# chenhuims/DistributedDeepLearningSpark

Measured on AMD Instinct MI355X. Metric: images/sec (whole node) ResNet-50 ImageNet-shape at 1/2/4/8 MI355X, higher is better.
Workload: dtype bf16; 1 GPU; model=resnet50, global_batch=256, image=224, per_gpu_batch=256, parallelism=dp1, optimizer=sgd-momentum, buckets=4

## Files before the change

distributeddeeplearningspark_amd/csrc/kernels/gemm_stream.hip:

```cpp
#include "ddl_gemm_kernel.h"

namespace ddl {
namespace gst {

constexpr int THREADS = 256;
constexpr int BM = 64;
constexpr int LDS_BUDGET = 80 * 1024;
typedef __attribute__((address_space(3))) void lds_t;

template <int WN, int K>
struct Cfg {
  static constexpr int NB = 4 * WN;
  static constexpr int RN = WN / 16;
  static constexpr int KS = K / 32;
  static constexpr int CPR = K / 8;
  static constexpr int TILE = BM * K * 2;
  static constexpr int D = TILE / 1024 / 4;
  static constexpr int OCPR = NB / 8;
  static constexpr int STAGE = BM * NB * 2;
  static constexpr int RPP = THREADS / OCPR;
  static constexpr int S = BM / RPP;
  static constexpr int NBUF_FIT = (LDS_BUDGET - STAGE) / TILE;
  static constexpr int NBUF = NBUF_FIT > 4 ? 4 : NBUF_FIT;
  static constexpr int LDS = NBUF * TILE + STAGE;
  static_assert(NBUF >= 2, "A ring needs two buffers");
  static_assert(D >= 1 && OCPR >= 8 && RPP >= 1 && BM % RPP == 0, "shape");
  static_assert((NBUF - 1) * (D + S) <= 63, "vmcnt range");
  static_assert(4 * 2 * OCPR * 8 * 4 <= STAGE, "stats reduction fits in the staging buffer");
};

template <int CPR>
__device__ __forceinline__ int sw(int r) {
  if constexpr (CPR == 8) return (r >> 1) & 7;
  else return r & 15;
}

template <int N>
__device__ __forceinline__ void wait_vm() {
  __builtin_amdgcn_s_waitcnt((N & 15) | ((N >> 4) << 14) | 0x0F70);
}

template <class CF>
__device__ __forceinline__ void wait_tile(int younger_store_tiles) {
  constexpr int base = (CF::NBUF - 1) * CF::D;
  switch (younger_store_tiles) {
    case 0: wait_vm<base>(); break;
    case 1: wait_vm<base + CF::S>(); break;
    case 2: wait_vm<base + 2 * CF::S>(); break;
    default: wait_vm<base + 3 * CF::S>(); break;
  }
}

template <class CF>
__device__ __forceinline__ void stage_a(const bf16_t* __restrict__ A, long lda, int M, int m0, char* slot, int w,
                                        int lane) {
#pragma unroll
  for (int i = 0; i < CF::D; ++i) {
    const int blk = i * 4 + w;
    const int u = blk * 64 + lane;
    const int r = u / CF::CPR, cp = u % CF::CPR;
    const int c = cp ^ sw<CF::CPR>(r);
    const int gr = min(m0 + r, M - 1);
    const bf16_t* src = A + (long)gr * lda + c * 8;
    const uint32_t dst = __builtin_amdgcn_readfirstlane((uint32_t) reinterpret_cast<uintptr_t>((lds_t*)(slot + blk * 1024)));
    asm volatile("s_mov_b32 m0, %1\n\tglobal_load_lds_dwordx4 %0, off" ::"v"(src), "s"(dst) : "memory", "m0");
  }
}

}

typedef __attribute__((ext_vector_type(2))) unsigned u32x2_t;
typedef __attribute__((ext_vector_type(4))) unsigned u32x4_t;
__device__ __forceinline__ u32x4_t ald128(const void* p) {
  u32x4_t v;
  asm volatile("global_load_dwordx4 %0, %1, off" : "=v"(v) : "v"(p) : "memory");
  return v;
}
__device__ __forceinline__ u32x2_t ald64(const void* p) {
  u32x2_t v;
  asm volatile("global_load_dwordx2 %0, %1, off" : "=v"(v) : "v"(p) : "memory");
  return v;
}
__device__ __forceinline__ unsigned ald32(const void* p) {
  unsigned v;
  asm volatile("global_load_dword %0, %1, off" : "=v"(v) : "v"(p) : "memory");
  return v;
}
__device__ __forceinline__ unsigned ald16(const void* p) {
  unsigned v;
  asm volatile("global_load_ushort %0, %1, off" : "=v"(v) : "v"(p) : "memory");
  return v;
}
__device__ __forceinline__ unsigned ald8(const void* p) {
  unsigned v;
  asm volatile("global_load_ubyte %0, %1, off" : "=v"(v) : "v"(p) : "memory");
  return v;
}
template <bool ASM> __device__ __forceinline__ u32x4_t sld128(const void* p) {
  if constexpr (ASM) return ald128(p);
  return *reinterpret_cast<const u32x4_t*>(p);
}
template <bool ASM> __device__ __forceinline__ u32x2_t sld64(const void* p) {
  if constexpr (ASM) return ald64(p);
  return *reinterpret_cast<const u32x2_t*>(p);
}
template <bool ASM> __device__ __forceinline__ unsigned sld32(const void* p) {
  if constexpr (ASM) return ald32(p);
  return *reinterpret_cast<const uint32_t*>(p);
}
template <bool ASM> __device__ __forceinline__ unsigned sld16(const void* p) {
  if constexpr (ASM) return ald16(p);
  return *reinterpret_cast<const uint16_t*>(p);
}
template <bool ASM> __device__ __forceinline__ unsigned sld8(const void* p) {
  if constexpr (ASM) return ald8(p);
  return *reinterpret_cast<const uint8_t*>(p);
}


template <int WN, int K, int BMODE, bool RES, int BNR = 0>
__global__ __launch_bounds__(gst::THREADS, 2) void gemm_stream_kernel(const GemmParams p) {
  using namespace gst;
  using CF = Cfg<WN, K>;
  constexpr bool kAsmSide = true;
  __shared__ __attribute__((aligned(16))) char smem[CF::LDS];
  char* const stg = smem + CF::NBUF * CF::TILE;
  const int lane = threadIdx.x & 63, w = threadIdx.x >> 6;
  const int n0 = blockIdx.y * CF::NB;
  const int mt = (p.M + BM - 1) / BM;
  const int nloc = ((int)blockIdx.x < mt) ? (mt - 1 - (int)blockIdx.x) / (int)gridDim.x + 1 : 0;
  const bf16_t* __restrict__ A = reinterpret_cast<const bf16_t*>(p.a);

  bf16x8 bfr[CF::RN][CF::KS];
  {
    const bf16_t* __restrict__ B = reinterpret_cast<const bf16_t*>(p.b);
#pragma unroll
    for (int rn = 0; rn < CF::RN; ++rn)
#pragma unroll
      for (int ks = 0; ks < CF::KS; ++ks) {
        const int n = n0 + WN * w + 16 * rn + (lane & 15);
        const int k = 32 * ks + 8 * (lane >> 4);
        if constexpr (BMODE == OP_KC) {
          bfr[rn][ks] = *reinterpret_cast<const bf16x8*>(B + (long)n * p.ldb + k);
        } else {
          s16x8 v;
#pragma unroll
          for (int j = 0; j < 8; ++j) v[j] = (short)B[(long)(k + j) * p.ldb + n];
          bfr[rn][ks] = __builtin_bit_cast(bf16x8, v);
        }
      }
  }
  float bias_r[CF::RN][4];
#pragma unroll
  for (int rn = 0; rn < CF::RN; ++rn) {
    const float4 bv = p.bias ? *reinterpret_cast<const float4*>(p.bias + n0 + WN * w + 16 * rn + 4 * (lane >> 4))
                             : make_float4(0.f, 0.f, 0.f, 0.f);
    bias_r[rn][0] = bv.x;
    bias_r[rn][1] = bv.y;
    bias_r[rn][2] = bv.z;
    bias_r[rn][3] = bv.w;
  }
  wait_vm<0>();
  auto tile_m0 = [&](int i) { return min((int)blockIdx.x + i * (int)gridDim.x, mt - 1) * BM; };

#pragma unroll
  for (int s = 0; s < CF::NBUF - 1; ++s) stage_a<CF>(A, p.lda, p.M, tile_m0(s), smem + s * CF::TILE, w, lane);

  float s1[8], s2[8];
#pragma unroll
  for (int e = 0; e < 8; ++e) s1[e] = s2[e] = 0.f;
  const int oc = threadIdx.x % CF::OCPR, orow = threadIdx.x / CF::OCPR;
  float bmu[8];
  float bsc[BNR == 2 ? 8 : 1], bsh[BNR == 2 ? 8 : 1];
  if constexpr (BNR != 0) {
    const float4 a = *reinterpret_cast<const float4*>(p.bnr_mean + n0 + oc * 8);
    const float4 b = *reinterpret_cast<const float4*>(p.bnr_mean + n0 + oc * 8 + 4);
    bmu[0] = a.x; bmu[1] = a.y; bmu[2] = a.z; bmu[3] = a.w;
    bmu[4] = b.x; bmu[5] = b.y; bmu[6] = b.z; bmu[7] = b.w;
  }
  if constexpr (BNR == 2) {
    const float4 a0 = *reinterpret_cast<const float4*>(p.bnr_scale + n0 + oc * 8);
    const float4 a1 = *reinterpret_cast<const float4*>(p.bnr_scale + n0 + oc * 8 + 4);
    const float4 b0 = *reinterpret_cast<const float4*>(p.bnr_shift + n0 + oc * 8);
    const float4 b1 = *reinterpret_cast<const float4*>(p.bnr_shift + n0 + oc * 8 + 4);
    bsc[0] = a0.x; bsc[1] = a0.y; bsc[2] = a0.z; bsc[3] = a0.w; bsc[4] = a1.x; bsc[5] = a1.y; bsc[6] = a1.z; bsc[7] = a1.w;
    bsh[0] = b0.x; bsh[1] = b0.y; bsh[2] = b0.z; bsh[3] = b0.w; bsh[4] = b1.x; bsh[5] = b1.y; bsh[6] = b1.z; bsh[7] = b1.w;
  }
  bf16_t* __restrict__ Cout = reinterpret_cast<bf16_t*>(p.c);

  for (int i = 0; i < nloc; ++i) {
    const int m0 = tile_m0(i);
    u32x2_t rres[BM / 16][CF::RN];
    unsigned rmk32[BM / 16];
    u32x2_t rmk64[CF::RN == 4 ? BM / 16 : 1];
    unsigned rodd_bits = 0u;
    const bool has_mask = p.resid_mask != nullptr;
    if constexpr (RES) {
#pragma unroll
      for (int mb = 0; mb < BM / 16; ++mb) {
        const int m = min(m0 + 16 * mb + (lane & 15), p.M - 1);
        long rrow = m;
        if (p.rsub_h) {
          int rn_, ri_, rj_;
          pix_decompose((uint32_t)m, p.rsub_h, p.rsub_w, rn_, ri_, rj_);
          const bool rodd = (ri_ | rj_) & 1;
          rodd_bits |= (rodd ? 1u : 0u) << mb;
// ... 77 lines not shown
          v[3] += (mk & 8u) ? __uint_as_float(rv.y & 0xffff0000u) : 0.f;
        }
        if (p.relu == ACT_RELU) {
#pragma unroll
          for (int e = 0; e < 4; ++e) v[e] = fmaxf(v[e], 0.f);
        }
        *reinterpret_cast<uint2*>(stg + r * (CF::NB * 2) + (((nl >> 3) ^ sw<CF::OCPR>(r)) << 4) + (nl & 7) * 2) =
            make_uint2(pack_bf16x2(v[0], v[1]), pack_bf16x2(v[2], v[3]));
      }
    }
    __builtin_amdgcn_s_waitcnt(0xC07F);
    __builtin_amdgcn_s_barrier();

    if constexpr (kAsmSide && BNR) {
      wait_vm<CF::D>();
      __builtin_amdgcn_sched_barrier(0);
#pragma unroll
      for (int ps = 0; ps < CF::S; ++ps) {
        asm volatile("" : "+v"(bx[ps]));
        if constexpr (BNR == 1) asm volatile("" : "+v"(bm8[ps]));
      }
    }
#pragma unroll
    for (int ps = 0; ps < CF::S; ++ps) {
      const int r = orow + ps * CF::RPP;
      const int m = m0 + r;
      const uint4 v = *reinterpret_cast<const uint4*>(stg + r * (CF::NB * 2) + ((oc ^ sw<CF::OCPR>(r)) << 4));
      if (m < p.M) {
        *reinterpret_cast<uint4*>(Cout + (long)m * p.ldc + n0 + oc * 8) = v;
        if constexpr (BNR) {
          const uint32_t wv[4] = {v.x, v.y, v.z, v.w};
          const uint32_t xv[4] = {bx[ps].x, bx[ps].y, bx[ps].z, bx[ps].w};
          uint32_t bmk = 0xffu;
          if constexpr (BNR == 1) bmk = p.bnr_mask ? bm8[ps] : 0xffu;
#pragma unroll
          for (int q = 0; q < 4; ++q) {
#pragma unroll
            for (int h = 0; h < 2; ++h) {
              const int e = 2 * q + h;
              const float xe = __uint_as_float(h ? (xv[q] & 0xffff0000u) : (xv[q] << 16));
              bool keep;
              if constexpr (BNR == 2) keep = xe * bsc[e] + bsh[e] > 0.f;
              else keep = (bmk >> e) & 1u;
              const float d = keep ? __uint_as_float(h ? (wv[q] & 0xffff0000u) : (wv[q] << 16)) : 0.f;
              s1[e] += d;
              s2[e] += d * (xe - bmu[e]);
            }
          }
        } else if (p.stats) {
          const uint32_t wv[4] = {v.x, v.y, v.z, v.w};
#pragma unroll
          for (int q = 0; q < 4; ++q) {
            const float lo = __uint_as_float(wv[q] << 16), hi = __uint_as_float(wv[q] & 0xffff0000u);
            s1[2 * q] += lo;
            s2[2 * q] += lo * lo;
            s1[2 * q + 1] += hi;
            s2[2 * q + 1] += hi * hi;
          }
        }
      }
    }
  }
  wait_vm<0>();

  if (p.stats) {
#pragma unroll
    for (int o = CF::OCPR; o < 64; o <<= 1)
#pragma unroll
      for (int e = 0; e < 8; ++e) {
        s1[e] += __shfl_xor(s1[e], o, 64);
        s2[e] += __shfl_xor(s2[e], o, 64);
      }
    __syncthreads();
    float* red = reinterpret_cast<float*>(stg);
    if (lane < CF::OCPR) {
#pragma unroll
      for (int e = 0; e < 8; ++e) {
        red[(w * CF::OCPR + lane) * 16 + e] = s1[e];
        red[(w * CF::OCPR + lane) * 16 + 8 + e] = s2[e];
      }
    }
    __syncthreads();
    float* st = p.stats + (long)(blockIdx.x % kStatShards) * 2 * p.N;
    for (int t = threadIdx.x; t < CF::NB; t += THREADS) {
      const int ch = t >> 3, e = t & 7;
      float a = 0.f, b = 0.f;
#pragma unroll
      for (int ww = 0; ww < 4; ++ww) {
        a += red[(ww * CF::OCPR + ch) * 16 + e];
        b += red[(ww * CF::OCPR + ch) * 16 + 8 + e];
      }
      atomicAdd(st + n0 + t, a);
      atomicAdd(st + p.N + n0 + t, b);
    }
  }
}

namespace {

int num_cus() {
  static int cus = 0;
  if (!cus) {
    int dev = 0;
    (void)hipGetDevice(&dev);
    if (hipDeviceGetAttribute(&cus, hipDeviceAttributeMultiprocessorCount, dev) != hipSuccess || cus <= 0) cus = 256;
  }
  return cus;
}

template <int WN, int K, int BMODE>
int launch_ws(const GemmParams& p, hipStream_t s) {
  using CF = gst::Cfg<WN, K>;
  constexpr bool kRes = !(WN == 64 && K == 128);
  constexpr bool kBnr = CF::NB <= (K >= 256 ? 64 : 128);
  const int panels = p.N / CF::NB;
  const int mt = (p.M + gst::BM - 1) / gst::BM;
  const int gx = std::max(1, std::min(mt, 2 * num_cus() / std::max(1, panels)));
  if (p.bnr_x && p.bnr_scale) {
    if constexpr (kBnr) {
      if (p.resid) return (int)hipErrorInvalidValue;
      hipLaunchKernelGGL((gemm_stream_kernel<WN, K, BMODE, false, 2>), dim3(gx, panels), dim3(gst::THREADS), 0, s, p);
    } else {
      return (int)hipErrorInvalidValue;
    }
  } else if (p.bnr_x) {
    if constexpr (kBnr && kRes) {
      if (p.resid)
        hipLaunchKernelGGL((gemm_stream_kernel<WN, K, BMODE, true, 1>), dim3(gx, panels), dim3(gst::THREADS), 0, s, p);
      else
        hipLaunchKernelGGL((gemm_stream_kernel<WN, K, BMODE, false, 1>), dim3(gx, panels), dim3(gst::THREADS), 0, s, p);
    } else if constexpr (kBnr) {
      if (p.resid) return (int)hipErrorInvalidValue;
      hipLaunchKernelGGL((gemm_stream_kernel<WN, K, BMODE, false, 1>), dim3(gx, panels), dim3(gst::THREADS), 0, s, p);
    } else {
      return (int)hipErrorInvalidValue;
    }
  } else if (p.resid) {
    if constexpr (kRes)
      hipLaunchKernelGGL((gemm_stream_kernel<WN, K, BMODE, true>), dim3(gx, panels), dim3(gst::THREADS), 0, s, p);
    else
      return (int)hipErrorInvalidValue;
  } else {
    hipLaunchKernelGGL((gemm_stream_kernel<WN, K, BMODE, false>), dim3(gx, panels), dim3(gst::THREADS), 0, s, p);
  }
  return (int)hipGetLastError();
}

template <int WN, int BMODE>
int launch_k(const GemmParams& p, hipStream_t s) {
  switch (p.K) {
    case 64: return launch_ws<WN, 64, BMODE>(p, s);
    case 128: return launch_ws<WN, 128, BMODE>(p, s);
    default:
      if constexpr (WN <= 32) return launch_ws<WN, 256, BMODE>(p, s);
      return (int)hipErrorInvalidValue;
  }
}

template <int BMODE>
int launch_panel(const GemmParams& p, int nb, hipStream_t s) {
  switch (nb) {
    case 64: return launch_k<16, BMODE>(p, s);
    case 128: return launch_k<32, BMODE>(p, s);
    default: return launch_k<64, BMODE>(p, s);
  }
}

}

int gemm_stream_panel(int N, int K) {
  if (K != 64 && K != 128 && K != 256) return 0;
  const int max_nb = K == 256 ? 128 : 256;
  for (int nb = max_nb; nb >= 64; nb >>= 1)
    if (N % nb == 0 && (N == nb || nb == max_nb)) return nb;
  return 0;
}

int launch_gemm_stream(const GemmParams& p, int epi, hipStream_t s) {
  int nb = gemm_stream_panel(p.N, p.K);
  if (p.resid && p.K == 128 && nb == 256) nb = 128;
  if (p.bnr_x && nb > (p.K >= 256 ? 64 : 128)) nb = p.K >= 256 ? 64 : 128;
  const bool ok = nb && epi == EPI_BF16 && p.a_mode == OP_KC && (p.b_mode == OP_KC || p.b_mode == OP_RC) &&
                  !p.om.enabled && !p.aux && !p.drop_thresh && (p.relu == ACT_NONE || p.relu == ACT_RELU) &&
                  p.beta == 0.f && p.k_split >= p.K && p.lda % 8 == 0 && p.ldc % 8 == 0 &&
                  (p.b_mode == OP_RC || p.ldb % 8 == 0) && (!p.resid || p.ldr % 4 == 0) &&
                  ((uintptr_t)p.a % 16 == 0) && ((uintptr_t)p.c % 16 == 0) &&
                  (p.b_mode == OP_RC || (uintptr_t)p.b % 16 == 0) && (!p.resid || (uintptr_t)p.resid % 8 == 0) &&
                  (!p.bnr_x || (p.stats && (uintptr_t)p.bnr_x % 16 == 0 && (uintptr_t)p.bnr_mean % 16 == 0)) &&
                  (!p.bnr_scale || (p.bnr_shift && !p.resid && (uintptr_t)p.bnr_scale % 16 == 0 &&
                                    (uintptr_t)p.bnr_shift % 16 == 0));
  if (!ok) return (int)hipErrorInvalidValue;
  return p.b_mode == OP_KC ? launch_panel<OP_KC>(p, nb, s) : launch_panel<OP_RC>(p, nb, s);
}

}
```

distributeddeeplearningspark_amd/ops/gemm.py:

```python
from __future__ import annotations

import math

import torch

from . import determinism as _det
from ._native import C

KC, RC, KC_GATHER, RC_GATHER, RC_TAPS, KC_GATHER8, RC_GATHER8 = 0, 1, 2, 3, 4, 5, 6
EPI_BF16, EPI_F32, EPI_F32_ATOMIC = 0, 1, 2
TILE256 = 4
TILE_STREAM = 5
TILE_CONV3 = 6
_TILES = {0: (128, 128), 1: (128, 64), 2: (64, 128), 3: (64, 64), TILE256: (256, 256), TILE_STREAM: (64, 256),
          TILE_CONV3: (224, 128)}
_ONE_PER_CU = (TILE256,)
_CU = 256
import os as _os

_USE256 = "auto"


_USE_STREAM = "1"
_TILE_FILL = 2.0
_WT_MIN_M = 4096
_LINEAR_WGRAD_ROUNDS = 1.0
_SPLIT_ROUNDS = 2.0


def stream_panel(N: int, K: int) -> int:
    if K not in (64, 128, 256):
        return 0
    max_nb = 128 if K == 256 else 256
    nb = max_nb
    while nb >= 64:
        if N % nb == 0 and (N == nb or nb == max_nb):
            return nb
        nb //= 2
    return 0


def use_stream(M, N, K, a_mode, b_mode, epi, lda, ldc, *, outmap=None, aux=None, drop_p=0.0, relu=0, beta=0.0,
               resid=None, ldr=0) -> bool:
    if _USE_STREAM == "0" or a_mode != KC or b_mode not in (KC, RC) or epi != EPI_BF16:
        return False
    if outmap is not None or aux is not None or drop_p or int(relu) > ACT_RELU or beta:
        return False
    if M < 16384 or not stream_panel(N, K) or lda % 8 or ldc % 8 or (resid is not None and ldr % 4):
        return False
    return True


def use_tile256(M: int, N: int, K: int, a_mode: int, b_mode: int, epi: int) -> bool:
    if _USE256 == "0" or a_mode > RC or b_mode > RC or K % 64 or M < 128 or N < 128:
        return False
    tiles = math.ceil(M / 256) * math.ceil(N / 256)
    if _USE256 == "1":
        return tiles >= _CU // 2
    return epi == EPI_BF16 and tiles >= 4 * _CU and K >= 4096


def choose_tile(M: int, N: int, bn_cap: int = 128) -> int:
    bn = 128 if (N > 64 and bn_cap >= 128) else 64
    bm = 128 if M > 64 else 64
    if bm == 128 and bn == 128 and math.ceil(M / 128) * math.ceil(N / 128) < _TILE_FILL * _CU:
        bm = 64 if M <= N else 128
        bn = 64 if M > N else 128
    for tid, (tm, tn) in _TILES.items():
        if (tm, tn) == (bm, bn):
            return tid
    return 3


def choose_split(M: int, N: int, K: int, tile: int, allow: bool, rounds: float | None = None) -> int:
    kfull = max(64, math.ceil(K / 64) * 64)
    if not allow:
        return kfull
    bm, bn = _TILES[tile]
    tiles = math.ceil(M / bm) * math.ceil(N / bn)
    per_cu = 1 if tile in _ONE_PER_CU else 2
    if tiles >= per_cu * _CU or K < 1024:
        return kfull
    splits = min(math.ceil((rounds or _SPLIT_ROUNDS) * per_cu * _CU / tiles), max(1, K // 512))
    ks = math.ceil(K / splits / 64) * 64
    return max(64, ks)


def gemm(a, b, c, M, N, K, a_mode, b_mode, lda, ldb, ldc, epi, *, alpha=1.0, beta=0.0, bias=None, resid=None,
         ldr=0, relu=False, geom=None, outmap=None, b_kdiv=0, b_tap_stride=0, stats=None, tile=None, k_split=None,
         bn_cap=128, aux=None, drop_p=0.0, drop_seed=0, split_rounds=None, resid_mask=None, bnr=None, rsub=None,
         slabs=None, defer_slabs=False):
    if tile is None:
        if use_stream(M, N, K, a_mode, b_mode, epi, lda, ldc, outmap=outmap, aux=aux, drop_p=drop_p, relu=relu,
                      beta=beta, resid=resid, ldr=ldr):
            tile = TILE_STREAM
        elif outmap is None and bnr is None and use_tile256(M, N, K, a_mode, b_mode, epi):
            tile = TILE256
        elif epi == EPI_F32 and a_mode <= RC and b_mode <= RC and big_wgrad(M, N, K) and _SPLITK_SLABS_MODE != "0":
            tile = 0
        else:
            tile = choose_tile(M, N, bn_cap)
    if (k_split is None and tile == 0 and epi == EPI_F32 and a_mode == RC and b_mode == RC and big_wgrad(M, N, K)
            and _SPLITK_SLABS_MODE == "auto" and slabs is not False):
        k_split = slab_split(M, N, K)
    if k_split is None:
        k_split = choose_split(M, N, K, tile, allow=(epi != EPI_BF16), rounds=split_rounds)
    split_stride = 0
    if k_split < K and epi != EPI_F32 and _det.enabled():
        k_split = max(64, math.ceil(K / 64) * 64)
    out, slab_beta = c, None
    if epi == EPI_F32 and k_split < K:
        if beta not in (0.0, 1.0):
            raise ValueError("split-K fp32 gemm supports beta in {0,1} (beta=0 needs a zeroed C)")
        auto = _SPLITK_SLABS_MODE == "auto" and tile == 0 and big_wgrad(M, N, K) and math.ceil(K / k_split) <= 32
        use_slabs = (_det.enabled() or _SPLITK_SLABS or auto) if slabs is None else (slabs or _det.enabled())
        if tile in (0, 1, 2, 3) + _ONE_PER_CU and use_slabs:
            splits = math.ceil(K / k_split)
            out, split_stride, slab_beta, ldc_c = _slab_workspace(splits * M * N, c.device), M * N, beta, ldc
            ldc, beta = N, 0.0
# ... 173 lines not shown
```

distributeddeeplearningspark_amd/csrc/kernels/conv3x3.hip:

```cpp
#include "ddl_gemm_kernel.h"
#include "ddl_ops.h"

namespace ddl {
namespace {

constexpr int C3_MAX_HALO_ROWS = 384;

struct Conv3Tiling {
  int img, rows, w;
  int P;
  int hh, ww;
  int hr, hr_pad;
  int tiles_img, tiles_row;
};

template <int BN, int EPI, int NB, int FR = 8>
__global__ __launch_bounds__(NTHREADS, 2) void conv3x3_halo_kernel(const GemmParams p, const Conv3Tiling t) {
  constexpr int RN = BN / 32;
  constexpr int B_BYTES = BN * BK * 2;
  extern __shared__ __attribute__((aligned(16))) char smem[];
  char* halo = smem;
  char* bring = smem + t.hr_pad * 128;

  const ConvGeom& g = p.g;
  const int H = g.hi, W = g.wi, C = g.c, N = g.n;
  const int tiles_n = (p.N + BN - 1) / BN;
  int bid, split;
  grid_tile(bid, split);
  const int tp = bid / tiles_n, tn = bid - tp * tiles_n;
  const int n0 = tn * BN;
  const int timg = tp / t.tiles_row, trow = tp - timg * t.tiles_row;
  const int img0 = timg * t.img, oy0 = trow * t.rows;
  const long m0 = ((long)img0 * H + oy0) * W;
  const int mend = (int)min((long)p.M, m0 + t.P);

  const int lane = threadIdx.x & 63, wid = threadIdx.x >> 6;
  const int wm = wid >> 1, wn = wid & 1;
  const int wn0 = wn * (BN / 2);

  int abase[FR];
#pragma unroll
  for (int i = 0; i < FR; ++i) {
    const int px = wm * (16 * FR) + 16 * i + (lane & 15);
    if (px < t.P) {
      const int im = px / (t.rows * t.w);
      const int rem = px - im * t.rows * t.w;
      const int oy = rem / t.w, ox = rem - oy * t.w;
      abase[i] = im * t.hh * t.ww + oy * t.ww + ox;
    } else {
      abase[i] = 0;
    }
  }

  Operand<BN, OP_KC> B;
  B.init(p.b, p.ldb, p.N, n0, p.K, g);

  const bf16_t* x = reinterpret_cast<const bf16_t*>(p.a);
  const int halo_instr = t.hr_pad / 32;
  constexpr int kMaxHaloInstr = C3_MAX_HALO_ROWS / 32;
  int hofs[kMaxHaloInstr];
#pragma unroll
  for (int j = 0; j < kMaxHaloInstr; ++j) {
    hofs[j] = -1;
    const int piece = wid + 4 * j;
    const int h = piece * 8 + (lane >> 3);
    if (j < halo_instr && h < t.hr) {
      const int chunk = (lane & 7) ^ (h & 6);
      const int im = h / (t.hh * t.ww);
      const int rem = h - im * t.hh * t.ww;
      const int hy = rem / t.ww, hx = rem - hy * t.ww;
      const int n = img0 + im, iy = oy0 + hy - 1, ix = hx - 1;
      if (n < N && (unsigned)iy < (unsigned)H && (unsigned)ix < (unsigned)W)
        hofs[j] = ((n * H + iy) * W + ix) * C + chunk * 8;
    }
  }
  const uint32_t halo_lds = lds_addr(halo) + (uint32_t)__builtin_amdgcn_readfirstlane(wid) * 1024u;
  auto stage_halo = [&](int kc) {
#pragma unroll
    for (int j = 0; j < kMaxHaloInstr; ++j) {
      if (j < halo_instr) {
        const void* src = hofs[j] >= 0 ? (const void*)(x + hofs[j] + kc * 64) : (const void*)ddl_zero_page;
        dma16(src, halo_lds + (uint32_t)(j * 4096));
      }
    }
  };
  auto stage_b = [&](int s, char* buf) {
    const int kc = s / 9, tap = s - kc * 9;
    B.dma(buf, tap * C + kc * 64, g, 0, 0, wid);
  };

  f32x4 acc[FR][RN];
#pragma unroll
  for (int i = 0; i < FR; ++i)
#pragma unroll
    for (int j = 0; j < RN; ++j) acc[i][j] = f32x4{0.f, 0.f, 0.f, 0.f};

  const int steps = (C / 64) * 9;
  stage_halo(0);
  stage_b(0, bring);
  for (int s = 0; s < steps; ++s) {
    const int kc = s / 9, tap = s - kc * 9;
    wait_vmcnt<0>();
    __builtin_amdgcn_s_barrier();
    if (s + 1 < steps) stage_b(s + 1, bring + ((s + 1) % NB) * B_BYTES);
    const char* lb = bring + (s % NB) * B_BYTES;
    const int r = tap / 3, c3 = tap - r * 3;
    const int toff = r * t.ww + c3;
#pragma unroll
    for (int kk = 0; kk < BK / 32; ++kk) {
      bf16x8 af[FR], bfr[RN];
#pragma unroll
      for (int j = 0; j < RN; ++j) bfr[j] = B.frag(lb, kk, j, wn0, lane);
#pragma unroll
      for (int i = 0; i < FR; ++i) {
        const int row = abase[i] + toff;
        const int ch = kk * 4 + (lane >> 4);
        af[i] = *reinterpret_cast<const bf16x8*>(halo + row * 128 + ((ch ^ (row & 6)) << 4));
      }
#pragma unroll
      for (int i = 0; i < FR; ++i)
#pragma unroll
        for (int j = 0; j < RN; ++j) acc[i][j] = mfma16x16x32(bfr[j], af[i], acc[i][j]);
    }
    if (NB == 2 || tap == 8) {
      asm volatile("s_waitcnt lgkmcnt(0)" ::: "memory");
      __builtin_amdgcn_s_barrier();
    }
    if (tap == 8 && s + 1 < steps) stage_halo(kc + 1);
  }

  gemm_epilogue<FR, RN, EPI>(p, acc, m0 + wm * (16 * FR), n0 + wn0, lane, bid, mend);
}

Conv3Tiling plan(const GemmParams& p, int max_px = 256) {
  const ConvGeom& g = p.g;
  Conv3Tiling t{};
  const int H = g.hi, W = g.wi;
  t.w = W;
  if (H * W <= max_px) {
    t.rows = H;
    t.img = std::max(1, std::min(max_px / (H * W), C3_MAX_HALO_ROWS / ((H + 2) * (W + 2))));
  } else {
    t.img = 1;
    t.rows = 0;
    for (int r = std::min(H, max_px / std::max(W, 1)); r >= 1; --r)
      if (H % r == 0 && (r + 2) * (W + 2) <= C3_MAX_HALO_ROWS) { t.rows = r; break; }
  }
  t.P = t.img * t.rows * t.w;
  t.hh = t.rows + 2;
  t.ww = W + 2;
  t.hr = t.img * t.hh * t.ww;
  t.hr_pad = (t.hr + 31) / 32 * 32;
  t.tiles_row = t.rows > 0 ? H / t.rows : 0;
  t.tiles_img = (g.n + t.img - 1) / t.img;
  return t;
}

template <int BN, int EPI, int NB, int FR>
int launch_fr(const GemmParams& p, const Conv3Tiling& t, hipStream_t s) {
  const int blocks = t.tiles_img * t.tiles_row * ((p.N + BN - 1) / BN);
  const size_t lds = (size_t)t.hr_pad * 128 + NB * BN * BK * 2;
  static bool attr = [] {
    return hipFuncSetAttribute(reinterpret_cast<const void*>(&conv3x3_halo_kernel<BN, EPI, NB, FR>),
                               hipFuncAttributeMaxDynamicSharedMemorySize,
                               C3_MAX_HALO_ROWS * 128 + NB * BN * BK * 2) == hipSuccess;
  }();
  (void)attr;
  hipLaunchKernelGGL((conv3x3_halo_kernel<BN, EPI, NB, FR>), dim3(blocks), dim3(NTHREADS), lds, s, p, t);
  return (int)hipGetLastError();
}

template <int BN, int EPI, int NB>
int launch(const GemmParams& p, const Conv3Tiling& t, hipStream_t s) {
  if (t.P <= 2 * 16 * 7) return launch_fr<BN, EPI, NB, 7>(p, t, s);
  return launch_fr<BN, EPI, NB, 8>(p, t, s);
}

struct WgradArgs {
  const bf16_t* dy;
  const bf16_t* x;
  float* out;
  int n, h, w, ci, co;
  int ntiles, tpb;
};

template <int WW, int SC, int KT>
__device__ __forceinline__ void wgrad_tile_mma(f32x4 (&acc)[9][2][2], const char* halo, const char* dyl,
                                               const int* hbt, const int (&ao)[2][2], const int boff, const int k1) {
  auto tr2 = [](const char* p1, const char* p2) {
    s16x4 lo = __builtin_amdgcn_ds_read_tr16_b64_v4i16((DDL_LDS s16x4*)p1);
    s16x4 hi = __builtin_amdgcn_ds_read_tr16_b64_v4i16((DDL_LDS s16x4*)p2);
    s16x8 r = {lo[0], lo[1], lo[2], lo[3], hi[0], hi[1], hi[2], hi[3]};
    return __builtin_bit_cast(bf16x8, r);
  };
  constexpr int JS = 2 * SC * 16;
  auto bload = [&](int r1, int r2, int tap, bf16x8 (&bf)[2]) {
    const int toff = ((tap / 3) * WW + (tap % 3)) * 16;
    const char* b1 = halo + boff + r1 * 16 + toff;
    const char* b2 = halo + boff + r2 * 16 + toff;
    bf[0] = tr2(b1, b2);
    bf[1] = tr2(b1 + JS, b2 + JS);
  };
  int hb1 = hbt[k1], hb2 = hbt[k1 + 4];
  const int k1n = (KT > 1 ? 32 : 0) + k1;
  int nhb1 = hbt[k1n], nhb2 = hbt[k1n + 4];
  bf16x8 af[2], bs[3][2];
  af[0] = tr2(dyl + ao[0][0], dyl + ao[0][1]);
  af[1] = tr2(dyl + ao[1][0], dyl + ao[1][1]);
  bload(hb1, hb2, 0, bs[0]);
  bload(hb1, hb2, 1, bs[1]);
#pragma unroll 1
  for (int kk = 0; kk < KT; ++kk) {
    const int kn = kk + 1 < KT ? kk + 1 : kk;
    const int kn2 = kk + 2 < KT ? kk + 2 : KT - 1;
    const int nnhb1 = hbt[kn2 * 32 + k1], nnhb2 = hbt[kn2 * 32 + k1 + 4];
    bf16x8 an[2];
#pragma unroll
    for (int tap = 0; tap < 9; ++tap) {
      if (tap + 2 <= 8) bload(hb1, hb2, tap + 2, bs[(tap + 2) % 3]);
      else bload(nhb1, nhb2, tap - 7, bs[(tap + 2) % 3]);
      if (tap == 7) {
        const char* ab = dyl + kn * 4096;
        an[0] = tr2(ab + ao[0][0], ab + ao[0][1]);
        an[1] = tr2(ab + ao[1][0], ab + ao[1][1]);
      }
#pragma unroll
      for (int i = 0; i < 2; ++i)
#pragma unroll
        for (int j = 0; j < 2; ++j) acc[tap][i][j] = mfma16x16x32(af[i], bs[tap % 3][j], acc[tap][i][j]);
      __builtin_amdgcn_sched_barrier(0);
    }
    af[0] = an[0];
    af[1] = an[1];
    hb1 = nhb1;
    hb2 = nhb2;
    nhb1 = nnhb1;
    nhb2 = nnhb2;
  }
}

template <int G, int KT>
constexpr int wgrad_lds_bytes() { return 8 * (64 * G + 4) * 16 + KT * 32 * 128 + KT * 32 * 4; }

template <int WW, int G, int KT, bool SLAB>
__global__ __launch_bounds__(NTHREADS, 2) void conv3x3_wgrad_kernel(const WgradArgs a, const Conv3Tiling t) {
  constexpr int SC = 64 * G + 4;
  extern __shared__ __attribute__((aligned(16))) char smem[];
  char* halo = smem;
  char* dyl = smem + 8 * SC * 16;
  int* hbt = reinterpret_cast<int*>(dyl + KT * 32 * 128);
  const int ci_tiles = a.ci / 64;
  int bid, split;
  grid_tile(bid, split);
  const int tco = bid / ci_tiles, tci = bid - tco * ci_tiles;
  const int co0 = tco * 64, ci0 = tci * 64;
  const int tp_beg = split * a.tpb, tp_end = min(a.ntiles, tp_beg + a.tpb);
  const int lane = threadIdx.x & 63, wid = threadIdx.x >> 6;
  const int wm0 = (wid >> 1) * 32, wn0 = (wid & 1) * 32;
// ... 333 lines not shown

template <bool SLAB>
int launch_wgrad(const WgradArgs& a, const Conv3Tiling& t, dim3 grid, bool pp, hipStream_t s) {
  switch (wgrad_variant(t)) {
    case 0: return launch_wgrad_v<58, 6, 7, SLAB>(a, t, grid, pp, s);
    case 1: return launch_wgrad_v<30, 5, 7, SLAB>(a, t, grid, pp, s);
    case 2: return launch_wgrad_v<16, 4, 7, SLAB>(a, t, grid, pp, s);
    case 3: return launch_wgrad_v<9, 6, 7, SLAB>(a, t, grid, pp, s);
    case 4: return launch_wgrad_v<10, 5, 6, SLAB>(a, t, grid, pp, s);
    case 5: return launch_wgrad_v<6, 6, 5, SLAB>(a, t, grid, pp, s);
    case 6: return launch_wgrad_v<4, 6, 3, SLAB>(a, t, grid, pp, s);
    case 7: return launch_wgrad_v<34, 4, 4, SLAB>(a, t, grid, pp, s);
    case 8: return launch_wgrad_v<18, 3, 4, SLAB>(a, t, grid, pp, s);
    default: return (int)hipErrorInvalidValue;
  }
}

}

bool conv3x3_wgrad_ok(int n, int h, int w, int ci, int co) {
  if (ci % 64 || co % 64 || n <= 0 || (long)n * h * w * std::max(ci, co) >= (1L << 31)) return false;
  GemmParams p{};
  p.g.n = n;
  p.g.hi = h;
  p.g.wi = w;
  const Conv3Tiling t = plan(p, kWgradPx);
  return t.rows > 0 && t.P >= 64 && t.P <= 256 && t.hr <= C3_MAX_HALO_ROWS && wgrad_variant(t) >= 0;
}

void conv3x3_wgrad_plan(int n, int h, int w, int ci, int co, int blocks_per_cu, int cus, int& splits, int& tpb,
                        int& ntiles) {
  GemmParams p{};
  p.g.n = n;
  p.g.hi = h;
  p.g.wi = w;
  const Conv3Tiling t = plan(p, kWgradPx);
  ntiles = t.tiles_img * t.tiles_row;
  const int pairs = (co / 64) * (ci / 64);
  const int want = std::max(1, (blocks_per_cu * cus + pairs - 1) / pairs);
  tpb = std::max(1, (ntiles + std::min(want, ntiles) - 1) / std::min(want, ntiles));
  splits = (ntiles + tpb - 1) / tpb;
}

int launch_conv3x3_wgrad(const bf16_t* dy, const bf16_t* x, float* gw, float* ws, int n, int h, int w, int ci, int co,
                         int splits, int tpb, bool pp, void* stream) {
  const hipStream_t s = reinterpret_cast<hipStream_t>(stream);
  GemmParams p{};
  p.g.n = n;
  p.g.hi = h;
  p.g.wi = w;
  const Conv3Tiling t = plan(p, kWgradPx);
  WgradArgs a{dy, x, ws ? ws : gw, n, h, w, ci, co, t.tiles_img * t.tiles_row, tpb};
  const dim3 grid((co / 64) * (ci / 64), splits);
  int rc = ws ? launch_wgrad<true>(a, t, grid, pp, s) : launch_wgrad<false>(a, t, grid, pp, s);
  if (rc || !ws) return rc;
  const long n4 = (long)co * 9 * ci / 4;
  const int per_group = (n4 >= 65536 || deterministic()) ? splits : 16;
  const dim3 rgrid((unsigned)((n4 + 255) / 256), (unsigned)((splits + per_group - 1) / per_group));
  hipLaunchKernelGGL(wgrad_slab_reduce_kernel, rgrid, dim3(256), 0, s, reinterpret_cast<const float4*>(ws), gw, n4,
                     splits, per_group);
  return (int)hipGetLastError();
}

bool conv3x3_halo_ok(const GemmParams& p) {
  const ConvGeom& g = p.g;
  if (p.a_mode != OP_KC_GATHER || p.b_mode != OP_KC || p.om.enabled || p.resid || p.aux || p.drop_thresh ||
      p.relu > ACT_RELU || p.k_split < p.K)
    return false;
  if (g.ntaps != 9 || g.sh != 1 || g.sw != 1 || g.hi != g.ho || g.wi != g.wo || g.c % 64 || g.c != g.tap_c ||
      p.N % 64 || p.K != 9 * g.c || p.ldc != p.N || p.ldb != p.K)
    return false;
  for (int r = 0; r < 3; ++r)
    for (int c = 0; c < 3; ++c)
      if (g.dh[r * 3 + c] != r - 1 || g.dw[r * 3 + c] != c - 1) return false;
  const Conv3Tiling t = plan(p);
  return t.rows > 0 && t.P >= 64 && t.hr <= C3_MAX_HALO_ROWS && p.M == g.n * g.hi * g.wi;
}

int launch_conv3x3(const GemmParams& p, int epi, hipStream_t s) {
  if (!conv3x3_halo_ok(p) || epi != EPI_BF16) return (int)hipErrorInvalidValue;
  const Conv3Tiling t = plan(p);
  const int tiles_px = t.tiles_img * t.tiles_row;
  const bool bn128 = p.N % 128 == 0 && (long)tiles_px * (p.N / 128) >= 2L * 256;
  if (p.bnr_x) return bn128 ? launch<128, EPI_BF16_BNR, 2>(p, t, s) : launch<64, EPI_BF16_BNR, 3>(p, t, s);
  if (bn128) return launch<128, EPI_BF16_LITE, 2>(p, t, s);
  return launch<64, EPI_BF16_LITE, 3>(p, t, s);
}

}
```

Before: 12780 images/sec.

## Add 8-wave one-workgroup-per-CU variant of the streaming GEMM for selected shapes

```diff
diff --git a/distributeddeeplearningspark_amd/csrc/kernels/gemm_stream.hip b/distributeddeeplearningspark_amd/csrc/kernels/gemm_stream.hip
--- a/distributeddeeplearningspark_amd/csrc/kernels/gemm_stream.hip
+++ b/distributeddeeplearningspark_amd/csrc/kernels/gemm_stream.hip
@@ -1,21 +1,25 @@
+#include <cstdlib>
+
 #include "ddl_gemm_kernel.h"
 
 namespace ddl {
 namespace gst {
 
-constexpr int THREADS = 256;
 constexpr int BM = 64;
-constexpr int LDS_BUDGET = 80 * 1024;
 typedef __attribute__((address_space(3))) void lds_t;
 
-template <int WN, int K>
+template <int WN, int K, int WV = 4>
 struct Cfg {
-  static constexpr int NB = 4 * WN;
+  static_assert(WV == 4 || WV == 8, "4 waves (two workgroups per CU) or 8 (one)");
+  static constexpr int WAVES = WV;
+  static constexpr int THREADS = 64 * WV;
+  static constexpr int LDS_BUDGET = WV * 20 * 1024;
+  static constexpr int NB = WV * WN;
   static constexpr int RN = WN / 16;
   static constexpr int KS = K / 32;
   static constexpr int CPR = K / 8;
   static constexpr int TILE = BM * K * 2;
-  static constexpr int D = TILE / 1024 / 4;
+  static constexpr int D = TILE / 1024 / WV;
   static constexpr int OCPR = NB / 8;
   static constexpr int STAGE = BM * NB * 2;
   static constexpr int RPP = THREADS / OCPR;
@@ -24,9 +28,9 @@
   static constexpr int NBUF = NBUF_FIT > 4 ? 4 : NBUF_FIT;
   static constexpr int LDS = NBUF * TILE + STAGE;
   static_assert(NBUF >= 2, "A ring needs two buffers");
-  static_assert(D >= 1 && OCPR >= 8 && RPP >= 1 && BM % RPP == 0, "shape");
+  static_assert(D >= 1 && D * WV * 1024 == TILE && OCPR >= 8 && RPP >= 1 && BM % RPP == 0, "shape");
   static_assert((NBUF - 1) * (D + S) <= 63, "vmcnt range");
-  static_assert(4 * 2 * OCPR * 8 * 4 <= STAGE, "stats reduction fits in the staging buffer");
+  static_assert(WV * 2 * OCPR * 8 * 4 <= STAGE, "stats reduction fits in the staging buffer");
 };
 
 template <int CPR>
@@ -56,7 +60,7 @@
                                         int lane) {
 #pragma unroll
   for (int i = 0; i < CF::D; ++i) {
-    const int blk = i * 4 + w;
+    const int blk = i * CF::WAVES + w;
     const int u = blk * 64 + lane;
     const int r = u / CF::CPR, cp = u % CF::CPR;
     const int c = cp ^ sw<CF::CPR>(r);
@@ -118,10 +122,10 @@
 }
 
 
-template <int WN, int K, int BMODE, bool RES, int BNR = 0>
-__global__ __launch_bounds__(gst::THREADS, 2) void gemm_stream_kernel(const GemmParams p) {
+template <int WN, int K, int BMODE, bool RES, int BNR = 0, int WV = 4>
+__global__ __launch_bounds__(64 * WV, WV == 4 ? 2 : 1) void gemm_stream_kernel(const GemmParams p) {
   using namespace gst;
-  using CF = Cfg<WN, K>;
+  using CF = Cfg<WN, K, WV>;
   constexpr bool kAsmSide = true;
   __shared__ __attribute__((aligned(16))) char smem[CF::LDS];
   char* const stg = smem + CF::NBUF * CF::TILE;
@@ -365,11 +369,11 @@
     }
     __syncthreads();
     float* st = p.stats + (long)(blockIdx.x % kStatShards) * 2 * p.N;
-    for (int t = threadIdx.x; t < CF::NB; t += THREADS) {
+    for (int t = threadIdx.x; t < CF::NB; t += CF::THREADS) {
       const int ch = t >> 3, e = t & 7;
       float a = 0.f, b = 0.f;
 #pragma unroll
-      for (int ww = 0; ww < 4; ++ww) {
+      for (int ww = 0; ww < WV; ++ww) {
         a += red[(ww * CF::OCPR + ch) * 16 + e];
         b += red[(ww * CF::OCPR + ch) * 16 + 8 + e];
       }
@@ -402,31 +406,89 @@
   if (p.bnr_x && p.bnr_scale) {
     if constexpr (kBnr) {
       if (p.resid) return (int)hipErrorInvalidValue;
-      hipLaunchKernelGGL((gemm_stream_kernel<WN, K, BMODE, false, 2>), dim3(gx, panels), dim3(gst::THREADS), 0, s, p);
+      hipLaunchKernelGGL((gemm_stream_kernel<WN, K, BMODE, false, 2>), dim3(gx, panels), dim3(CF::THREADS), 0, s, p);
     } else {
       return (int)hipErrorInvalidValue;
     }
   } else if (p.bnr_x) {
     if constexpr (kBnr && kRes) {
       if (p.resid)
-        hipLaunchKernelGGL((gemm_stream_kernel<WN, K, BMODE, true, 1>), dim3(gx, panels), dim3(gst::THREADS), 0, s, p);
+        hipLaunchKernelGGL((gemm_stream_kernel<WN, K, BMODE, true, 1>), dim3(gx, panels), dim3(CF::THREADS), 0, s, p);
       else
-        hipLaunchKernelGGL((gemm_stream_kernel<WN, K, BMODE, false, 1>), dim3(gx, panels), dim3(gst::THREADS), 0, s, p);
+        hipLaunchKernelGGL((gemm_stream_kernel<WN, K, BMODE, false, 1>), dim3(gx, panels), dim3(CF::THREADS), 0, s, p);
     } else if constexpr (kBnr) {
       if (p.resid) return (int)hipErrorInvalidValue;
-      hipLaunchKernelGGL((gemm_stream_kernel<WN, K, BMODE, false, 1>), dim3(gx, panels), dim3(gst::THREADS), 0, s, p);
+      hipLaunchKernelGGL((gemm_stream_kernel<WN, K, BMODE, false, 1>), dim3(gx, panels), dim3(CF::THREADS), 0, s, p);
     } else {
       return (int)hipErrorInvalidValue;
     }
   } else if (p.resid) {
     if constexpr (kRes)
-      hipLaunchKernelGGL((gemm_stream_kernel<WN, K, BMODE, true>), dim3(gx, panels), dim3(gst::THREADS), 0, s, p);
+      hipLaunchKernelGGL((gemm_stream_kernel<WN, K, BMODE, true>), dim3(gx, panels), dim3(CF::THREADS), 0, s, p);
     else
       return (int)hipErrorInvalidValue;
   } else {
-    hipLaunchKernelGGL((gemm_stream_kernel<WN, K, BMODE, false>), dim3(gx, panels), dim3(gst::THREADS), 0, s, p);
+    hipLaunchKernelGGL((gemm_stream_kernel<WN, K, BMODE, false>), dim3(gx, panels), dim3(CF::THREADS), 0, s, p);
   }
   return (int)hipGetLastError();
+}
+
+template <int WN, int K, int BMODE, bool RES, int BNR>
+int launch_wide_as(const GemmParams& p, hipStream_t s) {
+  using CF = gst::Cfg<WN, K, 8>;
+  static_assert(CF::LDS <= 160 * 1024, "one workgroup per CU");
+  const int panels = p.N / CF::NB;
+  const int mt = (p.M + gst::BM - 1) / gst::BM;
+  const int gx = std::max(1, std::min(mt, num_cus() / std::max(1, panels)));
+  hipLaunchKernelGGL((gemm_stream_kernel<WN, K, BMODE, RES, BNR, 8>), dim3(gx, panels), dim3(CF::THREADS), 0, s, p);
+  return (int)hipGetLastError();
+}
+
+template <int WN, int K, int BMODE>
+int launch_wide(const GemmParams& p, hipStream_t s) {
+  const bool bnr2 = p.bnr_x && p.bnr_scale, bnr1 = p.bnr_x && !p.bnr_scale;
+  if constexpr ((WN == 32 && K == 256) || (WN == 64 && K == 128)) {
+    if (!p.resid && !p.bnr_x) return launch_wide_as<WN, K, BMODE, false, 0>(p, s);
+  } else if constexpr (WN == 16 && K == 256) {
+    if (bnr2 && !p.resid) return launch_wide_as<WN, K, BMODE, false, 2>(p, s);
+    if (bnr1 && p.resid) return launch_wide_as<WN, K, BMODE, true, 1>(p, s);
+    if (bnr1) return launch_wide_as<WN, K, BMODE, false, 1>(p, s);
+    if (p.resid && !p.bnr_x) return launch_wide_as<WN, K, BMODE, true, 0>(p, s);
+  } else if constexpr (WN == 32 && (K == 128 || K == 64)) {
+    if (bnr1 && p.resid) return launch_wide_as<WN, K, BMODE, true, 1>(p, s);
+  }
+  return (int)hipErrorInvalidValue;
+}
+
+template <int BMODE>
+int launch_wide_panel(const GemmParams& p, int wn, hipStream_t s) {
+  if (p.K == 256) return wn == 32 ? launch_wide<32, 256, BMODE>(p, s) : launch_wide<16, 256, BMODE>(p, s);
+  if (p.K == 128) return wn == 64 ? launch_wide<64, 128, BMODE>(p, s) : launch_wide<32, 128, BMODE>(p, s);
+  return launch_wide<32, 64, BMODE>(p, s);
+}
+
+enum : int { WIDE_K256_PLAIN = 1, WIDE_K256_SIDE = 2, WIDE_K128_PLAIN = 4, WIDE_K128_RES_BNR = 8, WIDE_K64_RES_BNR = 16 };
+constexpr int kWideAdopted = WIDE_K256_SIDE | WIDE_K128_PLAIN | WIDE_K128_RES_BNR;
+
+int wide_mask() {
+  const char* e = std::getenv("DDL_STREAM_WIDE");
+  return (e && *e) ? (std::atoi(e) & 31) : kWideAdopted;
+}
+
+int wide_wn(int N, int K, bool resid, bool bnr1, bool bnr2) {
+  const int m = wide_mask();
+  const bool plain = !resid && !bnr1 && !bnr2;
+  if (K == 256) {
+    if (plain) return ((m & WIDE_K256_PLAIN) && N % 256 == 0) ? 32 : 0;
+    if (bnr2 && resid) return 0;
+    return ((m & WIDE_K256_SIDE) && N % 128 == 0) ? 16 : 0;
+  }
+  if (K == 128) {
+    if (plain) return ((m & WIDE_K128_PLAIN) && N % 512 == 0) ? 64 : 0;
+    return ((m & WIDE_K128_RES_BNR) && resid && bnr1 && N % 256 == 0) ? 32 : 0;
+  }
+  if (K == 64) return ((m & WIDE_K64_RES_BNR) && resid && bnr1 && N % 256 == 0) ? 32 : 0;
+  return 0;
 }
 
 template <int WN, int BMODE>
@@ -451,7 +513,9 @@
 
 }
 
-int gemm_stream_panel(int N, int K) {
+namespace {
+
+int panel4(int N, int K) {
   if (K != 64 && K != 128 && K != 256) return 0;
   const int max_nb = K == 256 ? 128 : 256;
   for (int nb = max_nb; nb >= 64; nb >>= 1)
@@ -459,8 +523,16 @@
   return 0;
 }
 
+}
+
+int gemm_stream_panel(int N, int K) {
+  const int nb = panel4(N, K);
+  const int wn = nb ? wide_wn(N, K, false, false, false) : 0;
+  return wn ? 8 * wn : nb;
+}
+
 int launch_gemm_stream(const GemmParams& p, int epi, hipStream_t s) {
-  int nb = gemm_stream_panel(p.N, p.K);
+  int nb = panel4(p.N, p.K);
   if (p.resid && p.K == 128 && nb == 256) nb = 128;
   if (p.bnr_x && nb > (p.K >= 256 ? 64 : 128)) nb = p.K >= 256 ? 64 : 128;
   const bool ok = nb && epi == EPI_BF16 && p.a_mode == OP_KC && (p.b_mode == OP_KC || p.b_mode == OP_RC) &&
@@ -473,6 +545,8 @@
                   (!p.bnr_scale || (p.bnr_shift && !p.resid && (uintptr_t)p.bnr_scale % 16 == 0 &&
                                     (uintptr_t)p.bnr_shift % 16 == 0));
   if (!ok) return (int)hipErrorInvalidValue;
+  if (const int wn = wide_wn(p.N, p.K, p.resid != nullptr, p.bnr_x && !p.bnr_scale, p.bnr_x && p.bnr_scale))
+    return p.b_mode == OP_KC ? launch_wide_panel<OP_KC>(p, wn, s) : launch_wide_panel<OP_RC>(p, wn, s);
   return p.b_mode == OP_KC ? launch_panel<OP_KC>(p, nb, s) : launch_panel<OP_RC>(p, nb, s);
 }
 
diff --git a/distributeddeeplearningspark_amd/ops/gemm.py b/distributeddeeplearningspark_amd/ops/gemm.py
--- a/distributeddeeplearningspark_amd/ops/gemm.py
+++ b/distributeddeeplearningspark_amd/ops/gemm.py
@@ -28,6 +28,19 @@
 _SPLIT_ROUNDS = 2.0
 
 
+_STREAM_WIDE_ADOPTED = 2 | 4 | 8
+
+
+def _stream_wide_mask() -> int:
+    e = _os.environ.get("DDL_STREAM_WIDE", "")
+    if not e:
+        return _STREAM_WIDE_ADOPTED
+    try:
+        return int(e) & 31
+    except ValueError:
+        return 0
+
+
 def stream_panel(N: int, K: int) -> int:
     if K not in (64, 128, 256):
         return 0
@@ -35,6 +48,10 @@
     nb = max_nb
     while nb >= 64:
         if N % nb == 0 and (N == nb or nb == max_nb):
+            if K == 256 and N % 256 == 0 and (_stream_wide_mask() & 1):
+                return 256
+            if K == 128 and N % 512 == 0 and (_stream_wide_mask() & 4):
+                return 512
             return nb
         nb //= 2
     return 0
```

Result: no change. 12870 images/sec, median of 6 (+0.7%).

## Pipeline 3x3 conv halo and weights in 32-channel chunks with async ring

Applied to the files above, without the earlier changes.

```diff
diff --git a/distributeddeeplearningspark_amd/csrc/kernels/conv3x3.hip b/distributeddeeplearningspark_amd/csrc/kernels/conv3x3.hip
--- a/distributeddeeplearningspark_amd/csrc/kernels/conv3x3.hip
+++ b/distributeddeeplearningspark_amd/csrc/kernels/conv3x3.hip
@@ -14,13 +14,36 @@
   int tiles_img, tiles_row;
 };
 
-template <int BN, int EPI, int NB, int FR = 8>
+constexpr int C3_KS = 32;
+constexpr int C3_RING = 4;
+constexpr int C3_AHEAD = 3;
+constexpr int C3_HALO_PIECES = C3_MAX_HALO_ROWS / 64;
+
+__device__ __forceinline__ void c3_wait_vm(int n) {
+  switch (n) {
+    case 0: wait_vmcnt<0>(); break;
+    case 1: wait_vmcnt<1>(); break;
+    case 2: wait_vmcnt<2>(); break;
+    case 3: wait_vmcnt<3>(); break;
+    case 4: wait_vmcnt<4>(); break;
+    case 5: wait_vmcnt<5>(); break;
+    case 6: wait_vmcnt<6>(); break;
+    default: wait_vmcnt<7>(); break;
+  }
+}
+
+__device__ __forceinline__ int c3_byte(int row, int chunk) { return row * 64 + ((chunk ^ ((row >> 1) & 3)) << 4); }
+
+template <int BN, int EPI, int FR = 8>
 __global__ __launch_bounds__(NTHREADS, 2) void conv3x3_halo_kernel(const GemmParams p, const Conv3Tiling t) {
   constexpr int RN = BN / 32;
-  constexpr int B_BYTES = BN * BK * 2;
+  constexpr int WI = BN / 64;
+  constexpr int W_BYTES = BN * C3_KS * 2;
+  static_assert(2 * WI + 3 <= 7, "c3_wait_vm covers vmcnt 0..7");
   extern __shared__ __attribute__((aligned(16))) char smem[];
+  const int slot_bytes = t.hr_pad * 64;
   char* halo = smem;
-  char* bring = smem + t.hr_pad * 128;
+  char* ring = smem + 2 * slot_bytes;
 
   const ConvGeom& g = p.g;
   const int H = g.hi, W = g.wi, C = g.c, N = g.n;
@@ -51,21 +74,20 @@
       abase[i] = 0;
     }
   }
-
-  Operand<BN, OP_KC> B;
-  B.init(p.b, p.ldb, p.N, n0, p.K, g);
+  int bbyte[RN];
+#pragma unroll
+  for (int j = 0; j < RN; ++j) bbyte[j] = c3_byte(wn0 + 16 * j + (lane & 15), lane >> 4);
 
   const bf16_t* x = reinterpret_cast<const bf16_t*>(p.a);
-  const int halo_instr = t.hr_pad / 32;
-  constexpr int kMaxHaloInstr = C3_MAX_HALO_ROWS / 32;
-  int hofs[kMaxHaloInstr];
-#pragma unroll
-  for (int j = 0; j < kMaxHaloInstr; ++j) {
+  const bf16_t* wgt = reinterpret_cast<const bf16_t*>(p.b);
+  const int halo_pieces = t.hr_pad / 64;
+  int hofs[C3_HALO_PIECES];
+#pragma unroll
+  for (int j = 0; j < C3_HALO_PIECES; ++j) {
     hofs[j] = -1;
-    const int piece = wid + 4 * j;
-    const int h = piece * 8 + (lane >> 3);
-    if (j < halo_instr && h < t.hr) {
-      const int chunk = (lane & 7) ^ (h & 6);
+    const int h = (wid + 4 * j) * 16 + (lane >> 2);
+    if (j < halo_pieces && h < t.hr) {
+      const int chunk = (lane & 3) ^ ((h >> 1) & 3);
       const int im = h / (t.hh * t.ww);
       const int rem = h - im * t.hh * t.ww;
       const int hy = rem / t.ww, hx = rem - hy * t.ww;
@@ -74,19 +96,25 @@
         hofs[j] = ((n * H + iy) * W + ix) * C + chunk * 8;
     }
   }
-  const uint32_t halo_lds = lds_addr(halo) + (uint32_t)__builtin_amdgcn_readfirstlane(wid) * 1024u;
-  auto stage_halo = [&](int kc) {
-#pragma unroll
-    for (int j = 0; j < kMaxHaloInstr; ++j) {
-      if (j < halo_instr) {
-        const void* src = hofs[j] >= 0 ? (const void*)(x + hofs[j] + kc * 64) : (const void*)ddl_zero_page;
-        dma16(src, halo_lds + (uint32_t)(j * 4096));
-      }
-    }
+  int wofs[WI];
+#pragma unroll
+  for (int v = 0; v < WI; ++v) {
+    const int row = (wid + 4 * v) * 16 + (lane >> 2);
+    wofs[v] = (n0 + row) * (int)p.ldb + ((lane & 3) ^ ((row >> 1) & 3)) * 8;
+  }
+  const uint32_t wave_lds = (uint32_t)__builtin_amdgcn_readfirstlane(wid) * 1024u;
+  const uint32_t halo_lds = lds_addr(halo) + wave_lds;
+  const uint32_t ring_lds = lds_addr(ring) + wave_lds;
+  auto stage_halo = [&](int j, int hc) {
+    const void* src = hofs[j] >= 0 ? (const void*)(x + hofs[j] + hc * C3_KS) : (const void*)ddl_zero_page;
+    dma16(src, halo_lds + (uint32_t)((hc & 1) * slot_bytes + j * 4096));
   };
-  auto stage_b = [&](int s, char* buf) {
-    const int kc = s / 9, tap = s - kc * 9;
-    B.dma(buf, tap * C + kc * 64, g, 0, 0, wid);
+  auto stage_w = [&](int hc, int tap) {
+    const uint32_t dst = ring_lds + (uint32_t)(((9 * hc + tap) % C3_RING) * W_BYTES);
+    int k0 = tap * C + hc * C3_KS;
+    asm volatile("" : "+s"(k0));
+#pragma unroll
+    for (int v = 0; v < WI; ++v) dma16(wgt + wofs[v] + k0, dst + (uint32_t)(v * 4096));
   };
 
   f32x4 acc[FR][RN];
@@ -95,38 +123,44 @@
 #pragma unroll
     for (int j = 0; j < RN; ++j) acc[i][j] = f32x4{0.f, 0.f, 0.f, 0.f};
 
-  const int steps = (C / 64) * 9;
-  stage_halo(0);
-  stage_b(0, bring);
-  for (int s = 0; s < steps; ++s) {
-    const int kc = s / 9, tap = s - kc * 9;
-    wait_vmcnt<0>();
-    __builtin_amdgcn_s_barrier();
-    if (s + 1 < steps) stage_b(s + 1, bring + ((s + 1) % NB) * B_BYTES);
-    const char* lb = bring + (s % NB) * B_BYTES;
-    const int r = tap / 3, c3 = tap - r * 3;
-    const int toff = r * t.ww + c3;
-#pragma unroll
-    for (int kk = 0; kk < BK / 32; ++kk) {
-      bf16x8 af[FR], bfr[RN];
-#pragma unroll
-      for (int j = 0; j < RN; ++j) bfr[j] = B.frag(lb, kk, j, wn0, lane);
-#pragma unroll
-      for (int i = 0; i < FR; ++i) {
-        const int row = abase[i] + toff;
-        const int ch = kk * 4 + (lane >> 4);
-        af[i] = *reinterpret_cast<const bf16x8*>(halo + row * 128 + ((ch ^ (row & 6)) << 4));
-      }
-#pragma unroll
-      for (int i = 0; i < FR; ++i)
-#pragma unroll
-        for (int j = 0; j < RN; ++j) acc[i][j] = mfma16x16x32(bfr[j], af[i], acc[i][j]);
-    }
-    if (NB == 2 || tap == 8) {
+  const int nh = C / C3_KS;
+#pragma unroll
+  for (int j = 0; j < C3_HALO_PIECES; ++j)
+    if (j < halo_pieces) stage_halo(j, 0);
+#pragma unroll
+  for (int s = 0; s < C3_AHEAD; ++s) stage_w(0, s);
+
+  for (int hc = 0; hc < nh; ++hc) {
+    const bool more = hc + 1 < nh;
+    const char* lh = halo + (hc & 1) * slot_bytes;
+#pragma unroll
+    for (int tap = 0; tap < 9; ++tap) {
+      int young = 0;
+#pragma unroll
+      for (int d = 1; d <= C3_AHEAD; ++d)
+        if (tap - d >= 0 && tap - d < C3_HALO_PIECES) young += (more && tap - d < halo_pieces) ? 1 : 0;
+      const int tiles_after = (more || tap + C3_AHEAD - 1 < 9) ? C3_AHEAD - 1 : 8 - tap;
+      c3_wait_vm(young + WI * tiles_after);
       asm volatile("s_waitcnt lgkmcnt(0)" ::: "memory");
       __builtin_amdgcn_s_barrier();
-    }
-    if (tap == 8 && s + 1 < steps) stage_halo(kc + 1);
+      if (tap + C3_AHEAD < 9) stage_w(hc, tap + C3_AHEAD);
+      else if (more) stage_w(hc + 1, tap + C3_AHEAD - 9);
+      if (tap < C3_HALO_PIECES)
+        if (more && tap < halo_pieces) stage_halo(tap, hc + 1);
+
+      const char* lb = ring + ((9 * hc + tap) % C3_RING) * W_BYTES;
+      int toff = (tap / 3) * t.ww + (tap % 3);
+      asm volatile("" : "+s"(toff));
+      bf16x8 af[FR], bfr[RN];
+#pragma unroll
+      for (int j = 0; j < RN; ++j) bfr[j] = *reinterpret_cast<const bf16x8*>(lb + bbyte[j]);
+#pragma unroll
+      for (int i = 0; i < FR; ++i) af[i] = *reinterpret_cast<const bf16x8*>(lh + c3_byte(abase[i] + toff, lane >> 4));
+#pragma unroll
+      for (int i = 0; i < FR; ++i)
+#pragma unroll
+        for (int j = 0; j < RN; ++j) acc[i][j] = mfma16x16x32(bfr[j], af[i], acc[i][j]);
+    }
   }
 
   gemm_epilogue<FR, RN, EPI>(p, acc, m0 + wm * (16 * FR), n0 + wn0, lane, bid, mend);
@@ -150,30 +184,30 @@
   t.hh = t.rows + 2;
   t.ww = W + 2;
   t.hr = t.img * t.hh * t.ww;
-  t.hr_pad = (t.hr + 31) / 32 * 32;
+  t.hr_pad = (t.hr + 63) / 64 * 64;
   t.tiles_row = t.rows > 0 ? H / t.rows : 0;
   t.tiles_img = (g.n + t.img - 1) / t.img;
   return t;
 }
 
-template <int BN, int EPI, int NB, int FR>
+template <int BN, int EPI, int FR>
 int launch_fr(const GemmParams& p, const Conv3Tiling& t, hipStream_t s) {
   const int blocks = t.tiles_img * t.tiles_row * ((p.N + BN - 1) / BN);
-  const size_t lds = (size_t)t.hr_pad * 128 + NB * BN * BK * 2;
+  const size_t lds = (size_t)t.hr_pad * 128 + C3_RING * BN * C3_KS * 2;
   static bool attr = [] {
-    return hipFuncSetAttribute(reinterpret_cast<const void*>(&conv3x3_halo_kernel<BN, EPI, NB, FR>),
+    return hipFuncSetAttribute(reinterpret_cast<const void*>(&conv3x3_halo_kernel<BN, EPI, FR>),
                                hipFuncAttributeMaxDynamicSharedMemorySize,
-                               C3_MAX_HALO_ROWS * 128 + NB * BN * BK * 2) == hipSuccess;
+                               C3_MAX_HALO_ROWS * 128 + C3_RING * BN * C3_KS * 2) == hipSuccess;
   }();
   (void)attr;
-  hipLaunchKernelGGL((conv3x3_halo_kernel<BN, EPI, NB, FR>), dim3(blocks), dim3(NTHREADS), lds, s, p, t);
+  hipLaunchKernelGGL((conv3x3_halo_kernel<BN, EPI, FR>), dim3(blocks), dim3(NTHREADS), lds, s, p, t);
   return (int)hipGetLastError();
 }
 
-template <int BN, int EPI, int NB>
+template <int BN, int EPI>
 int launch(const GemmParams& p, const Conv3Tiling& t, hipStream_t s) {
-  if (t.P <= 2 * 16 * 7) return launch_fr<BN, EPI, NB, 7>(p, t, s);
-  return launch_fr<BN, EPI, NB, 8>(p, t, s);
+  if (t.P <= 2 * 16 * 7) return launch_fr<BN, EPI, 7>(p, t, s);
+  return launch_fr<BN, EPI, 8>(p, t, s);
 }
 
 struct WgradArgs {
@@ -673,9 +707,9 @@
   const Conv3Tiling t = plan(p);
   const int tiles_px = t.tiles_img * t.tiles_row;
   const bool bn128 = p.N % 128 == 0 && (long)tiles_px * (p.N / 128) >= 2L * 256;
-  if (p.bnr_x) return bn128 ? launch<128, EPI_BF16_BNR, 2>(p, t, s) : launch<64, EPI_BF16_BNR, 3>(p, t, s);
-  if (bn128) return launch<128, EPI_BF16_LITE, 2>(p, t, s);
-  return launch<64, EPI_BF16_LITE, 3>(p, t, s);
-}
-
-}
+  if (p.bnr_x) return bn128 ? launch<128, EPI_BF16_BNR>(p, t, s) : launch<64, EPI_BF16_BNR>(p, t, s);
+  if (bn128) return launch<128, EPI_BF16_LITE>(p, t, s);
+  return launch<64, EPI_BF16_LITE>(p, t, s);
+}
+
+}
```

New measurement: 12540 images/sec before, 12530 images/sec after. About the same (-0.0%).
